# piyanon108/iGate4xSoftphoneDSP

Measured on AMD Instinct MI355X. Metric: Msamples/s G.711 decode+RMS, 65536ch@8kHz; %HBM roofline at 1/2/4/8 GPU, higher is better.
Workload: dtype u8

## Files before the change

### igate4xsoftphonedsp_amd/capi.py

```python
from __future__ import annotations

import ctypes as C
import os

import numpy as np

_PKG = os.path.dirname(os.path.abspath(__file__))
LIB_PATH = os.path.join(_PKG, "libigdsp.so")

ABI_VERSION = 3
PT_PCMU, PT_PCMA, PT_R2S = 0, 8, 123
SAMPLES_PER_FRAME = 160
MAX_PAYLOAD = 256
STAGE_DEPTH = 8
ENC_SUN16, ENC_G191 = 0, 1
FLAG_SILENT, FLAG_PROBE_D5, FLAG_CLIPPED, FLAG_EMPTY = 1, 2, 4, 8
FLAG_SATURATED = 0x10
BSS_VOTE_FRAMES = 10
PTT_RELEASE_FRAMES = 12
PTT_ON, PTT_PRESS, PTT_RELEASE, PTT_TAKEOVER = 1, 2, 4, 8
LINK_R2S_PERIOD_MS, LINK_MISS_TICKS = 200, 12
LINK_AUDIO_ON, LINK_AUDIO_OFF, LINK_MISSING, LINK_LATE, LINK_RECOVERED, LINK_CAME_UP = 1, 2, 4, 8, 0x10, 0x20
LINK_EVENT_DEFAULT = 0x37
LINK_UP, LINK_AUDIO, LINK_ALARMED = 1, 2, 4
# ... 72 lines not shown
RTP_V2, RTP_X, RTP_MARKER, RTP_ED137_OK, RTP_KEEPALIVE, RTP_METERED, RTP_RUNT, RTP_OVERSIZE = 1, 2, 4, 8, 16, 32, 64, 128
TX_CHAN = np.dtype(
    [("r2s_send_ms", "<u8"), ("ts", "<u4"), ("ssrc", "<u4"), ("keepalive_ms", "<i4"), ("packet_cnt", "<i4"), ("seq", "<u2"), ("pt", "u1"),
     ("first_r2s", "u1"), ("tx_slave", "u1"), ("rx_slave", "u1"), ("tx_slave_changed", "u1"), ("rx_slave_changed", "u1"),
     ("slave_count", "<i4"), ("ptt", "u1"), ("sql", "u1"), ("call_in", "u1"), ("call_recorder", "u1"), ("pttid", "u1"),
     ("pttpriority", "u1"), ("bssi", "u1"), ("calltype", "u1"), ("tx_run", "<i2"), ("level", "u1"), ("reserved0", "u1"),
     ("reserved", "<u4", (4,))],
    align=True,
)
TX_INFO = np.dtype([("ed137", "<u4"), ("size", "<u2"), ("flags", "u1"), ("level", "u1")], align=True)
TX_CT_IDLE, TX_CT_RX, TX_CT_TX = 1, 2, 4
TX_SENT, TX_KEEPALIVE_PT, TX_MARKER, TX_STALE_PAYLOAD, TX_LEVEL_VALID = 1, 2, 4, 8, 16
TX_CTL_PTT, TX_CTL_SQL, TX_CTL_MARK, TX_CTL_SET = 1, 2, 4, 0x80
TX_PACKET = np.dtype([("pkt", "<u8"), ("call_id", "<i4"), ("ed137", "<u4"), ("size", "<u2"), ("flags", "u1"), ("level", "u1")], align=True)
TX_MAX_N = 236
TX_SLOT = 256
AGGREGATE = np.dtype({
    "names": ["sumsq", "samples", "frames", "n_silent", "n_clipped", "byte_mean_sum", "peak_slot"],
    "formats": ["<u8", "<u8", "<u8", "<u8", "<u8", "<u8", ("<u8", (AGG_MAX_RANKS,))],
    "offsets": [128 * i for i in range(7)],
    "itemsize": 8 * AGG_WORDS,
})


class Level(C.Structure):
    _fields_ = [("byte_mean", C.c_uint8), ("flags", C.c_uint8), ("peak", C.c_uint16), ("rms", C.c_float),
                ("percent", C.c_int32), ("peak_hold", C.c_uint16), ("dropped", C.c_uint16), ("frames", C.c_uint32)]


class Window(C.Structure):
    _fields_ = [("gate_mode", C.c_uint32), ("probe_alarm", C.c_uint32), ("d_hold", C.c_void_p), ("d_gate", C.c_void_p),
                ("d_probe", C.c_void_p), ("d_work", C.c_void_p)]


class ChanProbe(C.Structure):
    _fields_ = [("run", C.c_uint32), ("alarms", C.c_uint32)]


IO_INPUT, IO_RECORD, IO_BULK = 0, 1, 2


class IoBuf(C.Structure):
    _fields_ = [("bytes", C.c_size_t), ("role", C.c_uint32), ("reserved", C.c_uint32), ("ptr", C.c_void_p)]


class IoReport(C.Structure):
    _fields_ = [("placed", C.c_uint32), ("bulk_spread", C.c_uint32), ("classes_found", C.c_uint32), ("chunks_explored", C.c_uint32),
                ("probes", C.c_uint32), ("reseeds", C.c_uint32), ("chunk_bytes", C.c_uint64), ("explored_bytes", C.c_uint64),
                ("probe_ms_same", C.c_float), ("probe_ms_other", C.c_float), ("setup_ms", C.c_float), ("settle_ms", C.c_float)]

    def as_dict(self):
        return {k: (round(getattr(self, k), 4) if isinstance(getattr(self, k), float) else getattr(self, k))
                for k, _ in self._fields_ if not k.startswith("reserved")}


class IgdspError(RuntimeError):
    def __init__(self, code: int, where: str, detail: str = ""):
        self.code = code
        super().__init__(f"{where} failed: {ERRORS.get(code, code)}" + (f" ({detail})" if detail else ""))


_vp, _u32, _u64, _i32, _int = C.c_void_p, C.c_uint32, C.c_uint64, C.c_int32, C.c_int
PROTOTYPES = [
    ("igdsp_abi_version", _int, []),
    ("igdsp_create", _int, [C.POINTER(_vp), _int, _u32]),
    ("igdsp_destroy", _int, [_vp]),
    ("igdsp_last_error", C.c_char_p, [_vp]),
    ("igdsp_device_info", _int, [_vp, C.POINTER(_int), C.POINTER(_int), C.c_char_p, C.c_size_t]),
    ("igdsp_map_call", _int, [_vp, _i32, _u32]),
    ("igdsp_unmap_call", _int, [_vp, _i32]),
    ("igdsp_on_rtp_frame", _int, [_vp, _i32, C.c_uint8, _vp, _u32]),
    ("igdsp_flush", _int, [_vp, C.POINTER(_u32)]),
    ("igdsp_flush_begin", _int, [_vp, C.POINTER(_u32)]),
    ("igdsp_flush_end", _int, [_vp, _int]),
    ("igdsp_set_ed137", _int, [_vp, _i32, _u32]),
    ("igdsp_set_gate_mode", _int, [_vp, _u32]),
    ("igdsp_get_probe", _int, [_vp, _u32, C.POINTER(ChanProbe)]),
    ("igdsp_poll", _int, [_vp, _u32, C.POINTER(Level)]),
    ("igdsp_poll_call", _int, [_vp, _i32, C.POINTER(Level)]),
    ("igdsp_reset_hold", _int, [_vp, _u32]),
    ("igdsp_get_hold", _int, [_vp, _u32, _vp]),
    ("igdsp_decode_meter", _int, [_vp, _vp, _vp, _vp, _u32, _u32, _u32, _vp, _vp, _vp, _u32, _vp]),
    ("igdsp_encode", _int, [_vp, _vp, _vp, _u32, _u32, _u32, _vp, _int, _vp]),
    ("igdsp_roundtrip_peakhold", _int, [_vp, _vp, _vp, _u32, _u32, _u32, _vp, _vp, _vp, _vp, _int, _vp]),
    ("igdsp_hold_update", _int, [_vp, _vp, _u32, _u32, _u32, _vp, _vp, _vp]),
    ("igdsp_hold_reset", _int, [_vp, _vp, _u32, _vp, _vp]),
    ("igdsp_agg_reset", _int, [_vp, _vp, _vp]),
    ("igdsp_depayload", _int, [_vp, _vp, _vp, _vp, _u32, _u32, _u32, _u32, _vp, _vp, _vp, _vp]),
    ("igdsp_decode_meter_rtp", _int, [_vp, _vp, _vp, _u32, _u32, _vp, _vp, _vp, _u32, _vp]),
    ("igdsp_decode_meter_packets", _int, [_vp, _vp, _vp, _vp, _u32, _u32, _u32, _u32, _vp, _vp, _vp, _u32, _vp]),
    ("igdsp_decode_meter_packets_mixed", _int, [_vp, _vp, _vp, _vp, _vp, _u32, _u32, _u32, _vp, _vp, _vp, _u32, _vp]),
    ("igdsp_window_work_bytes", C.c_size_t, [_u32]),
    ("igdsp_window_update", _int, [_vp, _vp, _vp, _vp, _u32, _u32, _u32, C.POINTER(Window), _vp]),
    ("igdsp_decode_meter_window", _int, [_vp, _u32, _vp, _vp, _vp, _vp, _u32, _u32, _u32, _u32, _vp, _vp, _vp, _u32, C.POINTER(Window), _vp]),
    ("igdsp_wav_expand", _int, [_vp, _vp, _u32, _u32, _u32, _u32, _vp, _u64, _vp]),
    ("igdsp_tx_chan_init", _int, [_vp, C.c_char_p, _int, C.c_uint8, _u32, C.c_uint16, _u32, _i32, _u64]),
    ("igdsp_tx_calltype_bits", _int, [C.c_char_p]),
    ("igdsp_tx_packetize", _int, [_vp, _vp, _vp, _vp, _u32, _u32, _u32, _u64, _u32, _vp, _vp, _vp, _u32, _vp, _vp, _int, _vp]),
    ("igdsp_tx_open", _int, [_vp, _i32, C.c_char_p, _int, _i32, _u64]),
    ("igdsp_tx_close", _int, [_vp, _i32]),
    ("igdsp_tx_set_ptt", _int, [_vp, _i32, _int, _int, _int]),
    ("igdsp_tx_set_sql", _int, [_vp, _i32, _int, _int, _i32]),
    ("igdsp_tx_set_ptt_id", _int, [_vp, _i32, _int]),
    ("igdsp_tx_set_slave", _int, [_vp, _i32, _int, _int]),
    ("igdsp_tx_set_recorder", _int, [_vp, _i32, _int]),
    ("igdsp_tx_set_calltype", _int, [_vp, _i32, C.c_char_p]),
# ... 448 lines not shown
        self._ck(self.L.igdsp_tx_results(self.h, C.byref(p), C.byref(n)), "igdsp_tx_results")
        if n.value == 0:
            return np.zeros(0, TX_PACKET), np.zeros((0, TX_SLOT), np.uint8)
        ent = np.frombuffer((C.c_uint8 * (n.value * TX_PACKET.itemsize)).from_address(p.value), TX_PACKET).copy()
        pk = np.frombuffer((C.c_uint8 * (n.value * TX_SLOT)).from_address(int(ent["pkt"][0])), np.uint8).reshape(n.value, TX_SLOT).copy()
        return ent, pk

    def tx_get_chan(self, call_id: int) -> np.ndarray:
        out = np.zeros((), TX_CHAN)
        self._ck(self.L.igdsp_tx_get_chan(self.h, call_id, out.ctypes.data_as(_vp)), "igdsp_tx_get_chan")
        return out

    def tx_counts(self, call_id: int):
        r, d = _u32(), _u32()
        self._ck(self.L.igdsp_tx_counts(self.h, call_id, C.byref(r), C.byref(d)), "igdsp_tx_counts")
        return r.value, d.value

    @staticmethod
    def window(hold, gate_mode=GATE_ALWAYS, gate=None, probe=None, work=None, probe_alarm=0) -> Window:
        w = Window(gate_mode, probe_alarm, _ptr(hold), _ptr(gate), _ptr(probe), _ptr(work))
        w._keep = (hold, gate, probe, work)
        return w

    def window_work_bytes(self, C_: int) -> int:
        return int(self.L.igdsp_window_work_bytes(C_))

    def window_update(self, stats, C_, F_, n, win: Window, info=None, length=None, stream=None):
        self._ck(self.L.igdsp_window_update(self.h, _ptr(stats), _ptr(info), _ptr(length), C_, F_, n, C.byref(win), stream), "igdsp_window_update")

    def decode_meter_window(self, layout, packets, sizes, codec, radio, C_, F_, stride, hdr, stats, win: Window, info=None, agg=None, rank=0, stream=None):
        self._ck(self.L.igdsp_decode_meter_window(self.h, layout, _ptr(packets), _ptr(sizes), _ptr(codec), _ptr(radio), C_, F_, stride, hdr,
                                                  _ptr(stats), _ptr(info), _ptr(agg), rank, C.byref(win), stream), "igdsp_decode_meter_window")

    def wav_expand(self, payload, C_, F_, n, files, file_stride, rate=8000, stream=None):
        self._ck(self.L.igdsp_wav_expand(self.h, _ptr(payload), C_, F_, n, rate, _ptr(files), file_stride, stream), "igdsp_wav_expand")

    def g726_reorder(self, d_in, d_out, n_bytes, mode, stream=None):
        self._ck(self.L.igdsp_g726_reorder(self.h, _ptr(d_in), _ptr(d_out), n_bytes, mode, stream), "igdsp_g726_reorder")

    def gen_uniform(self, out, n_bytes, seed=0x20241218, first_byte=0, stream=None):
        self._ck(self.L.igdsp_gen_uniform(self.h, _ptr(out), n_bytes, seed, first_byte, stream), "igdsp_gen_uniform")

    def stream_read(self, src, n_bytes, sink, stream=None):
        self._ck(self.L.igdsp_stream_read(self.h, _ptr(src), n_bytes, _ptr(sink), stream), "igdsp_stream_read")

    def dev_alloc(self, nbytes: int) -> int:
        p = _vp()
        self._ck(self.L.igdsp_dev_alloc(self.h, C.byref(p), nbytes), "igdsp_dev_alloc")
        return p.value

    def dev_free(self, ptr: int):
        self._ck(self.L.igdsp_dev_free(self.h, ptr), "igdsp_dev_free")

    def dev_memset(self, ptr, value: int, nbytes: int):
        self._ck(self.L.igdsp_dev_memset(self.h, _ptr(ptr), value, nbytes), "igdsp_dev_memset")

    def io_alloc(self, bufs, explore_limit_bytes: int = 0):
        arr = (IoBuf * len(bufs))()
        for a, (nb, role) in zip(arr, bufs):
            a.bytes, a.role = int(nb), int(role)
        st, rep = _vp(), IoReport()
        self._ck(self.L.igdsp_io_alloc(self.h, arr, len(bufs), explore_limit_bytes, C.byref(st), C.byref(rep)), "igdsp_io_alloc")
        return IoSet(self, st), [a.ptr for a in arr], rep.as_dict()

    def sync(self, stream=None):
        self._ck(self.L.igdsp_sync(self.h, stream), "igdsp_sync")

    def probe_placement(self, buf, n_bytes, out=None, reps=10, stream=None) -> float:
        ms = C.c_float(0)
        self._ck(self.L.igdsp_probe_placement(self.h, _ptr(buf), n_bytes, _ptr(out), reps, C.byref(ms), stream), "igdsp_probe_placement")
        return float(ms.value)

    def timer(self):
        return Timer(self)


class IoSet:

    def __init__(self, ctx: Context, handle):
        self.ctx, self.h = ctx, handle

    def close(self):
        if self.h and self.ctx.h:
            self.ctx.L.igdsp_io_free(self.ctx.h, self.h)
        self.h = None


class DevView:

    def __init__(self, ptr: int, nbytes: int):
        self.__cuda_array_interface__ = {"shape": (int(nbytes),), "typestr": "|u1", "data": (int(ptr), False), "version": 3, "strides": None}


def as_tensor(ptr: int, nbytes: int, dtype=None, shape=None):
    import torch

    t = torch.as_tensor(DevView(ptr, nbytes), device="cuda")
    if dtype is not None:
        t = t.view(dtype)
    return t.view(shape) if shape is not None else t


class Timer:
    def __init__(self, ctx: Context):
        self.ctx = ctx
        self.t = _vp()
# ... 18 lines not shown
```

### igate4xsoftphonedsp_amd/csrc/igdsp_capi_ctx.hip

```cpp
#include "igdsp_ctx.h"

#include <algorithm>
#include <atomic>
#include <cmath>
#include <cstdlib>
#include <cstring>
#include <mutex>
#include <new>
#include <vector>

using namespace igdsp;
using igdsp_rx::kSlot;
using igdsp_rx::kStageDepth;

extern "C" {

int igdsp_abi_version(void) { return IGDSP_ABI_VERSION; }

int igdsp_create(igdsp_ctx **out, int device, uint32_t max_channels)
{
    if (!out || max_channels == 0 || max_channels > (1u << 24)) return IGDSP_EINVAL;
    *out = nullptr;
    int count = 0;
    if (hipGetDeviceCount(&count) != hipSuccess || count <= 0 || device < 0 || device >= count) return IGDSP_ENODEV;
    hipDeviceProp_t prop;
    if (hipGetDeviceProperties(&prop, device) != hipSuccess) return IGDSP_ENODEV;
    if (std::strncmp(prop.gcnArchName, "gfx950", 6) != 0) return IGDSP_ENODEV;
    if (hipSetDevice(device) != hipSuccess) return IGDSP_ENODEV;

    igdsp_ctx *ctx = new (std::nothrow) igdsp_ctx();
    if (!ctx) return IGDSP_ENOMEM;
    ctx->device = device;
    ctx->cus = prop.multiProcessorCount;
    ctx->name = prop.name;
    ctx->max_channels = max_channels;
    ctx->direct = std::vector<std::atomic<uint32_t>>(kDirectCalls);
    for (auto &d : ctx->direct) d.store(kNoChan, std::memory_order_relaxed);
    const size_t max_frames = (size_t)max_channels * kStageDepth;
    ctx->up_bytes = igdsp_rx::upload_layout(max_frames, max_channels).total;
    bool ok = hipStreamCreateWithFlags(&ctx->stream, hipStreamNonBlocking) == hipSuccess;
    ok = ok && hipEventCreateWithFlags(&ctx->flush_done, hipEventDisableTiming) == hipSuccess;
    for (int i = 0; i < igdsp_rx::RingMem::kArrays; ++i)
        ok = ok && hipHostMalloc(ctx->ring.array(i), igdsp_rx::RingMem::bytes(max_channels, i), hipHostMallocDefault) == hipSuccess;
    if (ok) ctx->rx.init(max_channels, ctx->ring);
    ok = ok && hipHostMalloc((void **)&ctx->h_up, ctx->up_bytes, hipHostMallocDefault) == hipSuccess;
    for (uint32_t i = 0; i < 2; ++i) {
        igdsp_rx::Published &pb = ctx->pub.set(i);
        ok = ok && hipHostMalloc((void **)&pb.last, max_channels * sizeof(igdsp_frame_stats), hipHostMallocDefault) == hipSuccess;
        ok = ok && hipHostMalloc((void **)&pb.hold, max_channels * sizeof(igdsp_chan_hold), hipHostMallocDefault) == hipSuccess;
        ok = ok && hipHostMalloc((void **)&pb.probe, max_channels * sizeof(igdsp_chan_probe), hipHostMallocDefault) == hipSuccess;
    }
    ok = ok && hipMalloc((void **)&ctx->d_up, ctx->up_bytes) == hipSuccess;
    ok = ok && hipMalloc((void **)&ctx->d_stats, 2 * max_frames * sizeof(igdsp_frame_stats)) == hipSuccess;
    ok = ok && hipMalloc((void **)&ctx->d_last, max_channels * sizeof(igdsp_frame_stats)) == hipSuccess;
    ok = ok && hipMalloc((void **)&ctx->d_hold, max_channels * sizeof(igdsp_chan_hold)) == hipSuccess;
    ok = ok && hipMalloc((void **)&ctx->d_probe, max_channels * sizeof(igdsp_chan_probe)) == hipSuccess;
    ok = ok && hipMalloc((void **)&ctx->d_queues, kQueueRing * 32u * sizeof(uint32_t)) == hipSuccess;
    ok = ok && hipMemset(ctx->d_queues, 0, kQueueRing * 32u * sizeof(uint32_t)) == hipSuccess;
    ok = ok && hipMemset(ctx->d_last, 0, max_channels * sizeof(igdsp_frame_stats)) == hipSuccess;
    ok = ok && hipMemset(ctx->d_probe, 0, max_channels * sizeof(igdsp_chan_probe)) == hipSuccess;
    if (const char *e = std::getenv("IGDSP_GLOBAL_QUEUE")) ctx->global_queue = std::atoi(e) != 0;
    if (const char *e = std::getenv("IGDSP_IO_SPARE_CHUNKS")) ctx->io_spare_cap = (size_t)std::max(0, std::atoi(e));
    if (!ok) {
        igdsp_destroy(ctx);
        return IGDSP_ENOMEM;
    }
    if (init_device_attributes() != hipSuccess) {
        igdsp_destroy(ctx);
        return IGDSP_EDEVICE;
    }
    bool up = launch_hold_reset(ctx->d_hold, max_channels, nullptr, ctx->stream) == hipSuccess;
    for (uint32_t i = 0; i < 2; ++i) {
        igdsp_rx::Published &pb = ctx->pub.set(i);
        std::memset(pb.last, 0, max_channels * sizeof(igdsp_frame_stats));
        std::memset(pb.probe, 0, max_channels * sizeof(igdsp_chan_probe));
        up = up && hipMemcpyAsync(pb.hold, ctx->d_hold, max_channels * sizeof(igdsp_chan_hold), hipMemcpyDeviceToHost, ctx->stream) == hipSuccess;
    }
    if (!up || hipStreamSynchronize(ctx->stream) != hipSuccess) {
        igdsp_destroy(ctx);
        return IGDSP_EDEVICE;
    }
    ctx->pool = make_pool(max_channels);
    *out = ctx;
    return IGDSP_OK;
}

int igdsp_destroy(igdsp_ctx *ctx)
{
    if (!ctx) return IGDSP_OK;
    ctx->pool.reset();
    if (ctx->device >= 0) (void)hipSetDevice(ctx->device);
    igdsp_tx_drop(ctx);
    igdsp_io_drop_spares(ctx);
    if (ctx->stream) { (void)hipStreamSynchronize(ctx->stream); (void)hipStreamDestroy(ctx->stream); }
    if (ctx->flush_done) (void)hipEventDestroy(ctx->flush_done);
    for (int i = 0; i < igdsp_rx::RingMem::kArrays; ++i) if (*ctx->ring.array(i)) (void)hipHostFree(*ctx->ring.array(i));
    const igdsp_rx::Published &p0 = ctx->pub.set(0), &p1 = ctx->pub.set(1);
    void *hosts[] = {ctx->h_up, p0.last, p0.hold, p0.probe, p1.last, p1.hold, p1.probe};
    for (void *p : hosts) if (p) (void)hipHostFree(p);
    void *devs[] = {ctx->d_up, ctx->d_stats, ctx->d_last, ctx->d_hold, ctx->d_probe, ctx->d_queues, ctx->d_enc_tab[0], ctx->d_enc_tab[1]};
    for (void *p : devs) if (p) (void)hipFree(p);
    delete ctx;
    return IGDSP_OK;
}

const char *igdsp_last_error(const igdsp_ctx *ctx) { return ctx ? ctx->err.c_str() : ""; }

int igdsp_device_info(const igdsp_ctx *ctx, int *device, int *compute_units, char *name, size_t name_len)
{
    if (!ctx) return IGDSP_EINVAL;
    if (device) *device = ctx->device;
    if (compute_units) *compute_units = ctx->cus;
    if (name && name_len) { std::strncpy(name, ctx->name.c_str(), name_len - 1); name[name_len - 1] = 0; }
    return IGDSP_OK;
}
// ... 153 lines not shown
    igdsp_frame_stats s;
    uint16_t peak_hold = 0;
    ctx->pub.read([&](const igdsp_rx::Published &p) { s = p.last[channel]; peak_hold = p.hold[channel].peak_hold; });
    out->byte_mean = s.byte_mean;
    out->flags = s.flags;
    out->peak = s.peak;
    out->rms = s.rms;
    out->percent = (int32_t)(float)(((double)s.rms * 100.0) / (double)IGDSP_METER_FULL_SCALE);
    out->peak_hold = peak_hold;
    out->dropped = (uint16_t)std::min<uint32_t>(ctx->rx.frames_dropped(channel), 65535u);
    out->frames = ctx->rx.frames_seen(channel);
    return IGDSP_OK;
}

int igdsp_poll_call(igdsp_ctx *ctx, int32_t call_id, igdsp_level *out)
{
    if (!ctx || !out) return IGDSP_EINVAL;
    const uint32_t ch = lookup(ctx, call_id);
    if (ch == kNoChan) return IGDSP_ENOENT;
    return igdsp_poll(ctx, ch, out);
}

int igdsp_reset_hold(igdsp_ctx *ctx, uint32_t channel)
{
    if (!ctx) return IGDSP_EINVAL;
    if (channel != 0xFFFFFFFFu && channel >= ctx->max_channels) return IGDSP_ERANGE;
    std::lock_guard<std::mutex> g(ctx->flush_mu);
    if (int rc = flush_end_locked(ctx, 1)) return rc;
    HIP_TRY(ctx, hipSetDevice(ctx->device));
    const uint32_t c0 = (channel == 0xFFFFFFFFu) ? 0 : channel;
    const uint32_t cn = (channel == 0xFFFFFFFFu) ? ctx->max_channels : 1;
    HIP_TRY(ctx, launch_hold_reset(ctx->d_hold + c0, cn, nullptr, ctx->stream));
    HIP_TRY(ctx, hipMemcpyAsync(ctx->pub.back().hold + c0, ctx->d_hold + c0, cn * sizeof(igdsp_chan_hold), hipMemcpyDeviceToHost, ctx->stream));
    HIP_TRY(ctx, hipStreamSynchronize(ctx->stream));
    ctx->pub.rewrite_front([&](igdsp_rx::Published &front, const igdsp_rx::Published &back) {
        std::memcpy(front.hold + c0, back.hold + c0, cn * sizeof(igdsp_chan_hold));
    });
    return IGDSP_OK;
}

int igdsp_get_hold(igdsp_ctx *ctx, uint32_t channel, igdsp_chan_hold *out)
{
    if (!ctx || !out) return IGDSP_EINVAL;
    if (channel >= ctx->max_channels) return IGDSP_ERANGE;
    ctx->pub.read([&](const igdsp_rx::Published &p) { *out = p.hold[channel]; });
    return IGDSP_OK;
}

int igdsp_get_probe(igdsp_ctx *ctx, uint32_t channel, igdsp_chan_probe *out)
{
    if (!ctx || !out) return IGDSP_EINVAL;
    if (channel >= ctx->max_channels) return IGDSP_ERANGE;
    ctx->pub.read([&](const igdsp_rx::Published &p) { *out = p.probe[channel]; });
    return IGDSP_OK;
}

int igdsp_dev_alloc(igdsp_ctx *ctx, void **d_ptr, size_t bytes)
{
    if (!ctx || !d_ptr) return IGDSP_EINVAL;
    *d_ptr = nullptr;
    if (bytes == 0) return IGDSP_OK;
    if (hipSetDevice(ctx->device) != hipSuccess) return IGDSP_ENODEV;
    hipError_t e = hipMalloc(d_ptr, bytes);
    return e == hipSuccess ? IGDSP_OK : fail(ctx, IGDSP_ENOMEM, "hipMalloc", e);
}

int igdsp_dev_free(igdsp_ctx *ctx, void *d_ptr)
{
    if (!ctx) return IGDSP_EINVAL;
    if (!d_ptr) return IGDSP_OK;
    HIP_TRY(ctx, hipSetDevice(ctx->device));
    HIP_TRY(ctx, hipFree(d_ptr));
    return IGDSP_OK;
}

int igdsp_dev_alloc_far(igdsp_ctx *ctx, void **d_ptr, size_t bytes, const void *d_in, size_t in_bytes, uint32_t max_tries,
                        size_t spacer_bytes, float *ms_first, float *ms_kept)
{
    if (!ctx || !d_ptr || !d_in || bytes == 0 || in_bytes < 10240u || max_tries == 0) return IGDSP_EINVAL;
    *d_ptr = nullptr;
    if (hipSetDevice(ctx->device) != hipSuccess) return IGDSP_ENODEV;
    if (spacer_bytes == 0) spacer_bytes = (size_t)12 << 30;
    const size_t cand_bytes = std::max(bytes, in_bytes / 10u + 4096u);
    std::vector<void *> spacers;
    void *best = nullptr;
    float t_best = 0.f, t_first = 0.f;
    int rc = IGDSP_OK;
    for (uint32_t k = 0; k < max_tries; ++k) {
        if (k > 0) {
            void *sp = nullptr;
            if (hipMalloc(&sp, spacer_bytes) != hipSuccess) { (void)hipGetLastError(); break; }
            spacers.push_back(sp);
        }
        void *cand = nullptr;
        if (hipMalloc(&cand, cand_bytes) != hipSuccess) { (void)hipGetLastError(); break; }
        float ms = 0.f;
        rc = igdsp_probe_placement(ctx, d_in, in_bytes, cand, 6, &ms, nullptr);
        if (rc != IGDSP_OK) { (void)hipFree(cand); break; }
        if (k == 0) t_first = ms;
        if (best == nullptr || ms < t_best) {
            if (best) (void)hipFree(best);
            best = cand; t_best = ms;
        } else {
            (void)hipFree(cand);
        }
        if (t_best < 0.92f * t_first) break;
    }
    for (void *sp : spacers) (void)hipFree(sp);
    if (rc != IGDSP_OK) { if (best) (void)hipFree(best); return rc; }
    if (!best) return fail(ctx, IGDSP_ENOMEM, "igdsp_dev_alloc_far");
    *d_ptr = best;
    if (ms_first) *ms_first = t_first;
    if (ms_kept) *ms_kept = t_best;
    return IGDSP_OK;
}

int igdsp_copy_h2d(igdsp_ctx *ctx, void *d_dst, const void *h_src, size_t bytes)
{
    if (!ctx || (bytes && (!d_dst || !h_src))) return IGDSP_EINVAL;
    HIP_TRY(ctx, hipSetDevice(ctx->device));
    HIP_TRY(ctx, hipMemcpy(d_dst, h_src, bytes, hipMemcpyHostToDevice));
    return IGDSP_OK;
}

int igdsp_copy_d2h(igdsp_ctx *ctx, void *h_dst, const void *d_src, size_t bytes)
// ... 73 lines not shown
```

### igate4xsoftphonedsp_amd/csrc/igdsp_ctx.h

```cpp
#pragma once
#include "igdsp_args.h"
#include "igdsp_internal.h"
#include "igdsp_rxstage.h"
#include "igdsp_snappool.h"

#include <atomic>
#include <cstdio>
#include <mutex>
#include <string>
#include <unordered_map>
#include <vector>

namespace {
constexpr uint32_t kNoChan = 0xFFFFFFFFu;
constexpr int32_t kDirectCalls = 1 << 16;
}

struct igdsp_ctx {
    int device = -1;
    int cus = 0;
    std::string name;
    uint32_t max_channels = 0;
    hipStream_t stream = nullptr;
    int variant = 0;
    std::string err;

    struct IoRange { const char *base; size_t bytes; };
    std::vector<IoRange> spread_ranges;
    std::vector<hipMemGenericAllocationHandle_t> io_spare[4];
    size_t io_spare_chunk = 0;
    size_t io_spare_cap = 16;
    uint32_t io_epoch = 0;
    std::mutex io_mu;
    bool is_spread(const void *p)
    {
        std::lock_guard<std::mutex> g(io_mu);
        for (const auto &r : spread_ranges) if ((const char *)p >= r.base && (const char *)p < r.base + r.bytes) return true;
        return false;
    }

    std::vector<std::atomic<uint32_t>> direct;
    std::unordered_map<int32_t, uint32_t> far;
    std::mutex far_mu;

    igdsp_rx::RingMem ring;
    igdsp_rx::Stager rx;
    std::atomic<uint32_t> gate_mode{IGDSP_GATE_ALWAYS};

    uint8_t *h_up = nullptr, *d_up = nullptr;
    size_t up_bytes = 0;
    igdsp_frame_stats *d_stats = nullptr;
    igdsp_frame_stats *d_last = nullptr;
    igdsp_chan_hold *d_hold = nullptr;
    igdsp_chan_probe *d_probe = nullptr;
    igdsp_rx::PublishedSet pub;
    hipEvent_t flush_done = nullptr;
    bool flush_open = false;
    uint32_t flush_nch = 0;
    std::mutex flush_mu;

    std::unique_ptr<igdsp::SnapshotPool> pool;

    struct TxSide;
    std::atomic<TxSide *> tx{nullptr};
    std::mutex tx_init_mu;

    uint32_t *d_queues = nullptr;
    uint8_t *d_enc_tab[2] = {nullptr, nullptr};
    std::once_flag enc_once[2];
    hipStream_t queue_owner[64];
    uint32_t queue_launches[64];
    uint32_t queue_used = 0;
    uint32_t queue_hint = 0;
    std::atomic_flag queue_lk = ATOMIC_FLAG_INIT;
    bool global_queue = true;
};
namespace {
constexpr uint32_t kQueueRing = 64;
const hipStream_t kFreeQueue = reinterpret_cast<hipStream_t>(~(uintptr_t)0);
}

void igdsp_io_drop_spares(igdsp_ctx *ctx);
void igdsp_tx_drop(igdsp_ctx *ctx);

static inline uint32_t lookup(igdsp_ctx *ctx, int32_t call_id)
{
// ... 82 lines not shown
```

### igate4xsoftphonedsp_amd/csrc/igdsp_io.hip

```cpp
#include "igdsp_ctx.h"

#include <algorithm>
#include <chrono>
#include <thread>
#include <cmath>
#include <cstdlib>
#include <cstring>
#include <new>

using namespace igdsp;

struct igdsp_io_set {
    struct Map { void *va = nullptr; size_t bytes = 0; std::vector<hipMemGenericAllocationHandle_t> handles; std::vector<uint8_t> cls; };
    uint32_t epoch = 0;
    std::vector<Map> maps;
    std::vector<void *> plain;
    size_t chunk = 0;
    int device = 0;
};

namespace {

constexpr size_t kSrcChunks = 10;

struct Chunk {
    hipMemGenericAllocationHandle_t h{};
    float tA = -1.f;
    float tB = -1.f;
    bool used = false;
    bool mapped = false;
    bool in_src = false;
    int cls = -1;
};

struct Source { void *va = nullptr; size_t n = 0; std::vector<size_t> idx; };

struct Explorer {
    igdsp_ctx *ctx = nullptr;
    hipStream_t s = nullptr;
    size_t chunk = 0;
    size_t va_align = 0;
    hipMemAllocationProp prop{};
    hipMemAccessDesc acc{};
    void *cand_va = nullptr;
    bool debug = false;
    hipEvent_t ea = nullptr, eb = nullptr;
    std::vector<Chunk> chunks;
    std::vector<Source> sources;
    size_t limit_chunks = 0;
    size_t probe_n = 0;
    uint32_t probes = 0;

    bool open(igdsp_ctx *c, size_t n) { ctx = c; s = c->stream; probe_n = n; return hipEventCreate(&ea) == hipSuccess && hipEventCreate(&eb) == hipSuccess; }
    bool ensure(size_t idx)
    {
        while (chunks.size() <= idx) {
            if (chunks.size() >= limit_chunks) return false;
            Chunk c;
            if (hipMemCreate(&c.h, chunk, &prop, 0) != hipSuccess) { (void)hipGetLastError(); return false; }
            chunks.push_back(c);
        }
        return true;
    }
    void unmap_scratch(size_t idx)
    {
        if (chunks[idx].mapped) { (void)hipMemUnmap((char *)cand_va + idx * chunk, chunk); chunks[idx].mapped = false; }
    }
    bool time_pair(const void *rd, void *dst, float *ms)
    {
        hipError_t e = hipSuccess;
        for (int i = 0; i < 2 && e == hipSuccess; ++i) e = launch_stream_rw(cfg_of(ctx, s), rd, probe_n, dst, s);
        if (e == hipSuccess) e = hipEventRecord(ea, s);
        for (int i = 0; i < 4 && e == hipSuccess; ++i) e = launch_stream_rw(cfg_of(ctx, s), rd, probe_n, dst, s);
        if (e == hipSuccess) e = hipEventRecord(eb, s);
        if (e == hipSuccess) e = hipEventSynchronize(eb);
// ... 271 lines not shown
            P.b = cb; P.c = cc; P.split = true; P.thrB = thrB; P.thrC = thrC;
        }
        X.drop_source(srcB);
    }
    bool run(igdsp_ctx *ctx, igdsp_io_set *set, const IoKnobs &kn, size_t limit)
    {
        igdsp_io_drop_spares(ctx);
        { std::lock_guard<std::mutex> g(ctx->io_mu); set->epoch = ++ctx->io_epoch; ctx->io_spare_chunk = X.chunk; }
        X.limit_chunks = limit / X.chunk; X.debug = kn.debug;
        ok = hipMemAddressReserve(&X.cand_va, X.limit_chunks * X.chunk, X.va_align, nullptr, 0) == hipSuccess && X.open(ctx, probe_bytes(X.chunk));
        classify(L.bulk_chunks >= 4 && !kn.no_spread, ctx->io_spare_cap);
        R.chunks_explored = (uint32_t)X.chunks.size(); R.explored_bytes = (uint64_t)X.chunks.size() * X.chunk; R.probes = X.probes;
        (void)hipGetLastError();
        return ok;
    }
    void classify(bool want_spread, size_t spare_cap)
    {
        std::vector<size_t> first;
        for (size_t k = 0; k < kSrcChunks && ok; ++k) { ok = X.ensure(k); first.push_back(k); }
        ok = ok && X.make_source(first, &srcA);
        {
            float t = 0.f;
            if (ok && X.ensure(kSrcChunks)) { for (int k = 0; k < 28 && ok; ++k) ok = X.probe(kSrcChunks, X.sources[srcA], &t, "warm"); }
        }
        if (ok) survey(false);
        for (int attempt = 0; attempt < 2 && ok && tmax > 1.02f * tmin && tmax < kPure * tmin; ++attempt)
            if (!reseed_A()) break;
        R.probe_ms_same = tmax; R.probe_ms_other = tmin;
        if (!ok || !(tmax > kBimodal * tmin)) return;
        R.classes_found = 2;
        P.fast = kNear * tmin; P.slow = tmax / kNear;
        if (L.in_chunks > kSrcChunks) walk(0, L.in_chunks - kSrcChunks, [this](size_t i) { return !X.chunks[i].in_src && timeA(i) && X.chunks[i].tA > P.slow; }, P.a);
        const size_t outs = L.rec_chunks + L.bulk_chunks;
        walk(0, want_spread ? std::max<size_t>(outs + kSrcChunks, 4 * kSrcChunks) : outs, [this](size_t i) { return fast_A(i); }, P.b);
        if (ok && want_spread && P.b.size() >= kSrcChunks + outs - L.bulk_chunks / 2) split_BC();
        if (ok && !want_spread && spare_cap > 0) {
            const size_t need0 = (L.in_chunks > kSrcChunks ? L.in_chunks - kSrcChunks : 0) + spare_cap, need1 = L.rec_chunks + L.bulk_chunks + spare_cap;
            size_t cnt0 = 0, cnt1 = 0;
            for (const auto &c : X.chunks) if (!c.in_src && c.tA >= 0.f) { if (c.tA > P.slow) ++cnt0; else if (c.tA < P.fast) ++cnt1; }
            size_t budget = 4 * spare_cap;
            for (size_t k = 0; k < X.chunks.size() && ok && budget > 0 && (cnt0 < need0 || cnt1 < need1); ++k) {
                Chunk &c = X.chunks[k];
                if (c.in_src || c.tA >= 0.f) continue;
                if (!timeA(k)) break;
                --budget;
                if (c.tA > P.slow) ++cnt0; else if (c.tA < P.fast) ++cnt1;
            }
        }
        if (!ok) return;
        P.a.insert(P.a.begin(), X.sources[srcA].idx.begin(), X.sources[srcA].idx.end());
        X.drop_source(srcA);
    }
};
int plain_path(igdsp_ctx *ctx, igdsp_io_buf *bufs, uint32_t n_bufs, igdsp_io_set *set)
{
    for (uint32_t i = 0; i < n_bufs; ++i) {
        if (hipMalloc(&bufs[i].ptr, bufs[i].bytes) != hipSuccess) { (void)hipGetLastError(); bufs[i].ptr = nullptr; return fail(ctx, IGDSP_ENOMEM, "igdsp_io_alloc: hipMalloc"); }
        set->plain.push_back(bufs[i].ptr);
    }
    return IGDSP_OK;
}
int reserve_ranges(igdsp_ctx *ctx, const igdsp_io_buf *bufs, uint32_t n_bufs, size_t va_align, igdsp_io_set *set, Layout &L)
{
    const size_t chunk = set->chunk;
    set->maps.resize(n_bufs); L.nch.resize(n_bufs);
    for (uint32_t role = 0; role < 3; ++role)
        for (uint32_t i = 0; i < n_bufs; ++i) if (bufs[i].role == role) L.order.push_back(i);
    for (uint32_t i = 0; i < n_bufs; ++i) {
        L.nch[i] = (bufs[i].bytes + chunk - 1) / chunk;
        auto &m = set->maps[i];
        m.bytes = L.nch[i] * chunk;
        if (hipMemAddressReserve(&m.va, m.bytes, va_align, nullptr, 0) != hipSuccess) { (void)hipGetLastError(); m.va = nullptr; return fail(ctx, IGDSP_ENOMEM, "igdsp_io_alloc: hipMemAddressReserve"); }
        if (bufs[i].role == IGDSP_IO_INPUT) { L.in_chunks += L.nch[i]; L.in_bytes += bufs[i].bytes; if (L.in0 < 0 || L.nch[i] > L.nch[L.in0]) L.in0 = (int)i; continue; }
        if (L.out0 < 0) L.out0 = (int)i;
        if (bufs[i].role == IGDSP_IO_RECORD) L.rec_chunks += L.nch[i]; else L.bulk_chunks += L.nch[i];
    }
    return IGDSP_OK;
}
int publish(igdsp_ctx *ctx, igdsp_io_buf *bufs, uint32_t n_bufs, const igdsp_io_set *set, bool spread)
{
    for (uint32_t i = 0; i < n_bufs; ++i) bufs[i].ptr = set->maps[i].va;
    if (!spread) return IGDSP_OK;
    std::lock_guard<std::mutex> g(ctx->io_mu);
    for (uint32_t i = 0; i < n_bufs; ++i)
        if (bufs[i].role == IGDSP_IO_BULK) ctx->spread_ranges.push_back({(const char *)set->maps[i].va, set->maps[i].bytes});
    return IGDSP_OK;
}
constexpr int kNotServed = 1;
int from_spares(igdsp_ctx *ctx, igdsp_io_buf *bufs, uint32_t n_bufs, const Layout &L, igdsp_io_set *set, const hipMemAccessDesc &acc, igdsp_io_report &R)
{
    const bool want_spread = L.bulk_chunks >= 4;
    const size_t second = want_spread ? L.bulk_chunks / 2 : 0, first = L.rec_chunks + L.bulk_chunks - second;
    std::unique_lock<std::mutex> g(ctx->io_mu);
    auto &S = ctx->io_spare;
    if (ctx->io_spare_chunk != set->chunk || S[0].size() < L.in_chunks || S[1].size() + S[2].size() < first || S[3].size() < second) return kNotServed;
    const uint32_t epoch = ctx->io_epoch;
    const int pref = want_spread ? 2 : 1;
    for (uint32_t i : L.order) {
        auto &m = set->maps[i];
        const size_t h2 = (bufs[i].role == IGDSP_IO_BULK && want_spread) ? L.nch[i] / 2 : 0;
        for (size_t k = 0; k < L.nch[i]; ++k) {
            const int from = bufs[i].role == IGDSP_IO_INPUT ? 0 : (k >= L.nch[i] - h2 && !S[3].empty()) ? 3
                           : !S[pref].empty() ? pref : !S[3 - pref].empty() ? 3 - pref : 3;
            m.handles.push_back(S[from].back()); m.cls.push_back((uint8_t)from); S[from].pop_back();
        }
    }
// ... 70 lines not shown
        if (c.tA > P.slow) c.cls = 0;
        else if (c.tA < P.fast) c.cls = !P.split ? 1 : (c.tB > P.thrB ? 2 : ((c.tB >= 0.f && c.tB < P.thrC) ? 3 : -1));
    }
    std::lock_guard<std::mutex> g(ctx->io_mu);
    for (auto &c : X.chunks)
        if (!c.used && !c.in_src && c.cls >= 0 && ctx->io_spare[c.cls].size() < ctx->io_spare_cap) { ctx->io_spare[c.cls].push_back(c.h); c.used = true; }
}
bool map_fresh(igdsp_io_set::Map &m, size_t nch, size_t chunk, const hipMemAllocationProp &prop, const hipMemAccessDesc &acc)
{
    const size_t have = m.handles.size();
    std::vector<hipMemGenericAllocationHandle_t> hs;
    bool ok = true;
    hipMemGenericAllocationHandle_t h;
    for (size_t k = have; k < nch && ok; ++k) if ((ok = hipMemCreate(&h, chunk, &prop, 0) == hipSuccess)) hs.push_back(h);
    ok = ok && map_chunks(m, chunk, hs, have, acc);
    m.handles.insert(m.handles.end(), hs.begin(), hs.end());
    m.cls.resize(m.handles.size(), 255);
    return ok;
}
float settle_ref(Explorer &X, const Layout &L, const igdsp_io_set *set, size_t *n)
{
    if (L.in0 < 0 || L.out0 < 0) return 0.f;
    *n = std::min(X.probe_n, std::min(L.nch[L.in0] * set->chunk, 10 * (L.nch[L.out0] * set->chunk - 4096)) / 10240 * 10240);
    const size_t keep = X.probe_n; X.probe_n = *n;
    float t = 0.f, t_ref = 0.f;
    const void *rd = set->maps[L.in0].va; void *wr = set->maps[L.out0].va;
    if (*n >= ((size_t)256 << 20) && X.time_pair(rd, wr, &t) && X.time_pair(rd, wr, &t)) t_ref = t;
    X.probe_n = keep;
    return t_ref;
}
float settle(igdsp_ctx *ctx, const Layout &L, const igdsp_io_set *set, size_t n, float t_ref, size_t released_chunks, bool debug)
{
    Explorer Y;
    const auto w0 = std::chrono::steady_clock::now();
    if (Y.open(ctx, n)) {
        const float min_wait = std::min(6000.f, (float)((double)released_chunks * (double)set->chunk / 25e9 * 1e3));
        int quiet = 0;
        for (;;) {
            float t = 0.f; if (!Y.time_pair(set->maps[L.in0].va, set->maps[L.out0].va, &t)) break;
            quiet = t <= 1.012f * t_ref ? quiet + 1 : 0;
            const float waited = std::chrono::duration<float, std::milli>(std::chrono::steady_clock::now() - w0).count();
            if (debug) std::fprintf(stderr, "[igdsp_io] settle: %.4f ms against %.4f before the release (%.0f of >= %.0f ms)\n", t, t_ref, waited, min_wait);
            if ((quiet >= 2 && waited >= min_wait) || waited > 8000.f) break;
            std::this_thread::sleep_for(std::chrono::milliseconds(50));
        }
    }
    const float ms = std::chrono::duration<float, std::milli>(std::chrono::steady_clock::now() - w0).count();
    Y.cleanup();
    return ms;
}
int place(igdsp_ctx *ctx, igdsp_io_buf *bufs, uint32_t n_bufs, size_t explore_limit_bytes, const IoKnobs &kn, igdsp_io_set *set,
          Explorer &X, igdsp_io_report &R)
{
    int vmm = 0;
    if (hipDeviceGetAttribute(&vmm, hipDeviceAttributeVirtualMemoryManagementSupported, ctx->device) != hipSuccess) { (void)hipGetLastError(); vmm = 0; }
    if (!vmm || kn.plain) return plain_path(ctx, bufs, n_bufs, set);
    X.prop.type = hipMemAllocationTypePinned; X.prop.location.type = hipMemLocationTypeDevice; X.prop.location.id = ctx->device;
    X.acc.location = X.prop.location; X.acc.flags = hipMemAccessFlagsProtReadWrite;
    size_t gran = 0;
    if (hipMemGetAllocationGranularity(&gran, &X.prop, hipMemAllocationGranularityRecommended) != hipSuccess || gran == 0) { (void)hipGetLastError(); return plain_path(ctx, bufs, n_bufs, set); }
    const size_t chunk = (((size_t)128 << 20) + gran - 1) / gran * gran;
    X.chunk = set->chunk = R.chunk_bytes = chunk;
    X.va_align = kn.align_mib >= 0 ? (size_t)kn.align_mib << 20 : chunk;
    Layout L;
    if (const int rc = reserve_ranges(ctx, bufs, n_bufs, X.va_align, set, L)) return rc;
    size_t free_b = 0, total_b = 0; (void)hipMemGetInfo(&free_b, &total_b);
    const double frac = kn.frac_set ? kn.limit_frac : (L.bulk_chunks >= 4 ? 0.85 : 0.5);
    const size_t limit = std::min(explore_limit_bytes ? explore_limit_bytes : (size_t)(frac * (double)free_b), (size_t)(0.9 * (double)free_b));
    const bool want_place = L.in_bytes >= ((size_t)512 << 20) && ((L.rec_chunks + L.bulk_chunks) > 0 || L.in_chunks > kSrcChunks) && limit / chunk >= 4 * kSrcChunks;
    const int spared = want_place ? from_spares(ctx, bufs, n_bufs, L, set, X.acc, R) : kNotServed;
    if (spared != kNotServed) return spared;
    Search S{X, L, kn.stride, R};
    bool ok = !want_place || S.run(ctx, set, kn, limit);
    if (ok && (!S.P.b.empty() || (L.rec_chunks + L.bulk_chunks == 0 && !S.P.a.empty()))) ok = hand_out(X, S.P, bufs, n_bufs, L, set, R);
    size_t settle_n = 0;
    const float t_ref = R.placed ? settle_ref(X, L, set, &settle_n) : 0.f;
    if (R.placed) keep_spares(ctx, X, S.P);
    const size_t released_chunks = (size_t)std::count_if(X.chunks.begin(), X.chunks.end(), [](const Chunk &c) { return !c.used; });
    X.cleanup();
    for (uint32_t i : L.order)
        if (ok && set->maps[i].handles.size() < L.nch[i]) ok = map_fresh(set->maps[i], L.nch[i], chunk, X.prop, X.acc);
    if (!ok) { (void)hipGetLastError(); return fail(ctx, IGDSP_ENOMEM, "igdsp_io_alloc: mapping chunks"); }
    publish(ctx, bufs, n_bufs, set, R.bulk_spread);
    if (kn.settle && t_ref > 0.f) R.settle_ms = settle(ctx, L, set, settle_n, t_ref, released_chunks, kn.debug);
    if (kn.debug && R.placed) { Explorer Y; if (Y.open(ctx, probe_bytes(chunk))) debug_check(Y, bufs, n_bufs, L, set, true); Y.cleanup(); }
    return IGDSP_OK;
}

}

void igdsp_io_drop_spares(igdsp_ctx *ctx)
{
    std::vector<hipMemGenericAllocationHandle_t> gone;
    std::unique_lock<std::mutex> g(ctx->io_mu);
    for (auto &v : ctx->io_spare) { gone.insert(gone.end(), v.begin(), v.end()); v.clear(); }
    g.unlock();
    for (auto h : gone) (void)hipMemRelease(h);
    (void)hipGetLastError();
}

extern "C" {

int igdsp_io_free(igdsp_ctx *ctx, igdsp_io_set *set)
{
    if (!ctx) return IGDSP_EINVAL;
    if (!set) return IGDSP_OK;
    (void)hipSetDevice(set->device);
    (void)hipDeviceSynchronize();
    {
        std::lock_guard<std::mutex> g(ctx->io_mu);
        for (auto &m : set->maps)
            for (size_t k = 0; k < ctx->spread_ranges.size();)
                if (ctx->spread_ranges[k].base == (const char *)m.va) ctx->spread_ranges.erase(ctx->spread_ranges.begin() + (long)k); else ++k;
    }
    for (auto &m : set->maps) {
        if (!m.va) continue;
        for (size_t i = 0; i < m.handles.size(); ++i) (void)hipMemUnmap((char *)m.va + i * set->chunk, set->chunk);
        std::vector<hipMemGenericAllocationHandle_t> gone;
        std::unique_lock<std::mutex> g(ctx->io_mu);
        for (size_t i = 0; i < m.handles.size(); ++i) {
            const uint8_t c = i < m.cls.size() ? m.cls[i] : 255;
            if (c < 4 && set->epoch == ctx->io_epoch && set->chunk == ctx->io_spare_chunk && ctx->io_spare[c].size() < ctx->io_spare_cap) ctx->io_spare[c].push_back(m.handles[i]);
            else gone.push_back(m.handles[i]);
        }
        g.unlock();
        for (auto h : gone) (void)hipMemRelease(h);
    }
    for (void *p : set->plain) if (p) (void)hipFree(p);
    (void)hipGetLastError();
    delete set;
    return IGDSP_OK;
}

int igdsp_internal_vmm_remap_check(igdsp_ctx *ctx, int mode, int *bytes)
{
    if (!ctx || !bytes) return IGDSP_EINVAL;
    HIP_TRY(ctx, hipSetDevice(ctx->device));
    hipMemAllocationProp prop{};
    prop.type = hipMemAllocationTypePinned;
    prop.location.type = hipMemLocationTypeDevice;
    prop.location.id = ctx->device;
    hipMemAccessDesc acc{};
    acc.location = prop.location;
    acc.flags = hipMemAccessFlagsProtReadWrite;
    size_t gran = 0;
    HIP_TRY(ctx, hipMemGetAllocationGranularity(&gran, &prop, hipMemAllocationGranularityRecommended));
    const size_t sz = std::max<size_t>(gran, (size_t)64 << 20);
    hipMemGenericAllocationHandle_t X, Y;
    void *v = nullptr, *wx = nullptr, *wy = nullptr;
    HIP_TRY(ctx, hipMemCreate(&X, sz, &prop, 0));
    HIP_TRY(ctx, hipMemCreate(&Y, sz, &prop, 0));
    HIP_TRY(ctx, hipMemAddressReserve(&v, sz, 0, nullptr, 0));
    HIP_TRY(ctx, hipMemAddressReserve(&wx, sz, 0, nullptr, 0));
    HIP_TRY(ctx, hipMemAddressReserve(&wy, sz, 0, nullptr, 0));
// ... 59 lines not shown
```

Before: 5.993 million.

## Route large dev_alloc buffers through VMM chunk placement search

Large allocations made with igdsp_dev_alloc (at least one 128 MiB chunk) now go through the same VMM physical-chunk placement machinery used by io_alloc. Chunks come from the spare pool by class, or from a fresh probe search, and are mapped into a contiguous VA range; freeing returns the handles to the spare pool. The aim is to place bulk buffers in physical memory classes with better HBM bandwidth, rather than wherever hipMalloc puts them. The cost is setup time for probing and settling, added complexity, and a fallback to hipMalloc when placement fails.

```diff
diff --git a/igate4xsoftphonedsp_amd/capi.py b/igate4xsoftphonedsp_amd/capi.py
--- a/igate4xsoftphonedsp_amd/capi.py
+++ b/igate4xsoftphonedsp_amd/capi.py
@@ -148,6 +148,14 @@
     def as_dict(self):
         return {k: (round(getattr(self, k), 4) if isinstance(getattr(self, k), float) else getattr(self, k))
                 for k, _ in self._fields_ if not k.startswith("reserved")}
+
+
+class DevAllocInfo(C.Structure):
+    _fields_ = [("placed", C.c_uint32), ("reason", C.c_uint32), ("cls", C.c_uint32), ("epoch", C.c_uint32), ("chunks", C.c_uint32),
+                ("from_spares", C.c_uint32), ("probes", C.c_uint32), ("classes_found", C.c_uint32), ("chunk_bytes", C.c_uint64),
+                ("explored_bytes", C.c_uint64), ("setup_ms", C.c_float), ("settle_ms", C.c_float)]
+    REASONS = ("placed", "small", "off", "no_vmm", "no_class", "vmm_failed")
+    as_dict = IoReport.as_dict
 
 
 class IgdspError(RuntimeError):
@@ -702,6 +710,13 @@
     def dev_free(self, ptr: int):
         self._ck(self.L.igdsp_dev_free(self.h, ptr), "igdsp_dev_free")
 
+    def dev_alloc_info(self, ptr: int) -> dict:
+        fn = self.L.igdsp_internal_dev_alloc_info
+        fn.restype, fn.argtypes = _int, [_vp, _vp, C.POINTER(DevAllocInfo)]
+        info = DevAllocInfo()
+        self._ck(fn(self.h, ptr, C.byref(info)), "igdsp_internal_dev_alloc_info")
+        return dict(info.as_dict(), reason=DevAllocInfo.REASONS[info.reason])
+
     def dev_memset(self, ptr, value: int, nbytes: int):
         self._ck(self.L.igdsp_dev_memset(self.h, _ptr(ptr), value, nbytes), "igdsp_dev_memset")
 
diff --git a/igate4xsoftphonedsp_amd/csrc/igdsp_capi_ctx.hip b/igate4xsoftphonedsp_amd/csrc/igdsp_capi_ctx.hip
--- a/igate4xsoftphonedsp_amd/csrc/igdsp_capi_ctx.hip
+++ b/igate4xsoftphonedsp_amd/csrc/igdsp_capi_ctx.hip
@@ -61,6 +61,7 @@
     ok = ok && hipMemset(ctx->d_probe, 0, max_channels * sizeof(igdsp_chan_probe)) == hipSuccess;
     if (const char *e = std::getenv("IGDSP_GLOBAL_QUEUE")) ctx->global_queue = std::atoi(e) != 0;
     if (const char *e = std::getenv("IGDSP_IO_SPARE_CHUNKS")) ctx->io_spare_cap = (size_t)std::max(0, std::atoi(e));
+    if (const char *e = std::getenv("IGDSP_DEV_ALLOC_PLACE")) ctx->dev_place = std::atoi(e) != 0;
     if (!ok) {
         igdsp_destroy(ctx);
         return IGDSP_ENOMEM;
@@ -320,25 +321,6 @@
     if (!ctx || !out) return IGDSP_EINVAL;
     if (channel >= ctx->max_channels) return IGDSP_ERANGE;
     ctx->pub.read([&](const igdsp_rx::Published &p) { *out = p.probe[channel]; });
-    return IGDSP_OK;
-}
-
-int igdsp_dev_alloc(igdsp_ctx *ctx, void **d_ptr, size_t bytes)
-{
-    if (!ctx || !d_ptr) return IGDSP_EINVAL;
-    *d_ptr = nullptr;
-    if (bytes == 0) return IGDSP_OK;
-    if (hipSetDevice(ctx->device) != hipSuccess) return IGDSP_ENODEV;
-    hipError_t e = hipMalloc(d_ptr, bytes);
-    return e == hipSuccess ? IGDSP_OK : fail(ctx, IGDSP_ENOMEM, "hipMalloc", e);
-}
-
-int igdsp_dev_free(igdsp_ctx *ctx, void *d_ptr)
-{
-    if (!ctx) return IGDSP_EINVAL;
-    if (!d_ptr) return IGDSP_OK;
-    HIP_TRY(ctx, hipSetDevice(ctx->device));
-    HIP_TRY(ctx, hipFree(d_ptr));
     return IGDSP_OK;
 }
 
diff --git a/igate4xsoftphonedsp_amd/csrc/igdsp_ctx.h b/igate4xsoftphonedsp_amd/csrc/igdsp_ctx.h
--- a/igate4xsoftphonedsp_amd/csrc/igdsp_ctx.h
+++ b/igate4xsoftphonedsp_amd/csrc/igdsp_ctx.h
@@ -16,6 +16,28 @@
 constexpr int32_t kDirectCalls = 1 << 16;
 }
 
+#define IGDSP_DEV_PLACED        0u
+#define IGDSP_DEV_SMALL         1u
+#define IGDSP_DEV_OFF           2u
+#define IGDSP_DEV_NO_VMM        3u
+#define IGDSP_DEV_NO_CLASS      4u
+#define IGDSP_DEV_VMM_FAILED    5u
+struct igdsp_dev_alloc_info {
+    uint32_t placed;
+    uint32_t reason;
+    uint32_t cls;
+    uint32_t epoch;
+    uint32_t chunks;
+    uint32_t from_spares;
+    uint32_t probes;
+    uint32_t classes_found;
+    uint64_t chunk_bytes;
+    uint64_t explored_bytes;
+    float setup_ms;
+    float settle_ms;
+};
+extern "C" int igdsp_internal_dev_alloc_info(igdsp_ctx *ctx, const void *d_ptr, igdsp_dev_alloc_info *out);
+
 struct igdsp_ctx {
     int device = -1;
     int cus = 0;
@@ -32,6 +54,16 @@
     size_t io_spare_cap = 16;
     uint32_t io_epoch = 0;
     std::mutex io_mu;
+    struct DevAlloc {
+        size_t chunk = 0;
+        std::vector<hipMemGenericAllocationHandle_t> handles;
+        uint32_t epoch = 0;
+        igdsp_dev_alloc_info info{};
+    };
+    std::unordered_map<const void *, DevAlloc> dev_allocs;
+    bool dev_place = true;
+    int dev_last_cls = -1;
+    uint32_t dev_last_epoch = 0;
     bool is_spread(const void *p)
     {
         std::lock_guard<std::mutex> g(io_mu);
diff --git a/igate4xsoftphonedsp_amd/csrc/igdsp_io.hip b/igate4xsoftphonedsp_amd/csrc/igdsp_io.hip
--- a/igate4xsoftphonedsp_amd/csrc/igdsp_io.hip
+++ b/igate4xsoftphonedsp_amd/csrc/igdsp_io.hip
@@ -21,6 +21,8 @@
 
 namespace {
 
+constexpr size_t kChunkBytes = (size_t)128 << 20;
+constexpr size_t kDevPlaceMinBytes = kChunkBytes;
 constexpr size_t kSrcChunks = 10;
 
 struct Chunk {
@@ -398,6 +400,19 @@
         X.drop_source(srcA);
     }
 };
+bool open_vmm(igdsp_ctx *ctx, const IoKnobs &kn, Explorer &X)
+{
+    int vmm = 0;
+    if (hipDeviceGetAttribute(&vmm, hipDeviceAttributeVirtualMemoryManagementSupported, ctx->device) != hipSuccess) { (void)hipGetLastError(); vmm = 0; }
+    if (!vmm) return false;
+    X.prop.type = hipMemAllocationTypePinned; X.prop.location.type = hipMemLocationTypeDevice; X.prop.location.id = ctx->device;
+    X.acc.location = X.prop.location; X.acc.flags = hipMemAccessFlagsProtReadWrite;
+    size_t gran = 0;
+    if (hipMemGetAllocationGranularity(&gran, &X.prop, hipMemAllocationGranularityRecommended) != hipSuccess || gran == 0) { (void)hipGetLastError(); return false; }
+    X.chunk = (kChunkBytes + gran - 1) / gran * gran;
+    X.va_align = kn.align_mib >= 0 ? (size_t)kn.align_mib << 20 : X.chunk;
+    return true;
+}
 int plain_path(igdsp_ctx *ctx, igdsp_io_buf *bufs, uint32_t n_bufs, igdsp_io_set *set)
 {
     for (uint32_t i = 0; i < n_bufs; ++i) {
@@ -574,16 +589,8 @@
 int place(igdsp_ctx *ctx, igdsp_io_buf *bufs, uint32_t n_bufs, size_t explore_limit_bytes, const IoKnobs &kn, igdsp_io_set *set,
           Explorer &X, igdsp_io_report &R)
 {
-    int vmm = 0;
-    if (hipDeviceGetAttribute(&vmm, hipDeviceAttributeVirtualMemoryManagementSupported, ctx->device) != hipSuccess) { (void)hipGetLastError(); vmm = 0; }
-    if (!vmm || kn.plain) return plain_path(ctx, bufs, n_bufs, set);
-    X.prop.type = hipMemAllocationTypePinned; X.prop.location.type = hipMemLocationTypeDevice; X.prop.location.id = ctx->device;
-    X.acc.location = X.prop.location; X.acc.flags = hipMemAccessFlagsProtReadWrite;
-    size_t gran = 0;
-    if (hipMemGetAllocationGranularity(&gran, &X.prop, hipMemAllocationGranularityRecommended) != hipSuccess || gran == 0) { (void)hipGetLastError(); return plain_path(ctx, bufs, n_bufs, set); }
-    const size_t chunk = (((size_t)128 << 20) + gran - 1) / gran * gran;
-    X.chunk = set->chunk = R.chunk_bytes = chunk;
-    X.va_align = kn.align_mib >= 0 ? (size_t)kn.align_mib << 20 : chunk;
+    if (kn.plain || !open_vmm(ctx, kn, X)) return plain_path(ctx, bufs, n_bufs, set);
+    const size_t chunk = set->chunk = R.chunk_bytes = X.chunk;
     Layout L;
     if (const int rc = reserve_ranges(ctx, bufs, n_bufs, X.va_align, set, L)) return rc;
     size_t free_b = 0, total_b = 0; (void)hipMemGetInfo(&free_b, &total_b);
@@ -609,6 +616,130 @@
     return IGDSP_OK;
 }
 
+constexpr int8_t kDevNext[5][4] = {{0, 2, 1, 3}, {2, 1, 3, -1}, {0, -1, -1, -1}, {3, 0, -1, -1}, {0, 2, -1, -1}};
+
+void dev_unmap(void *va, size_t n, size_t chunk)
+{
+    for (size_t k = 0; k < n; ++k) (void)hipMemUnmap((char *)va + k * chunk, chunk);
+    (void)hipGetLastError();
+}
+void dev_give_back(igdsp_ctx *ctx, const igdsp_ctx::DevAlloc &d)
+{
+    std::vector<hipMemGenericAllocationHandle_t> gone;
+    {
+        std::lock_guard<std::mutex> g(ctx->io_mu);
+        const uint32_t c = d.info.cls;
+        for (auto h : d.handles) {
+            if (c < 4 && d.epoch == ctx->io_epoch && d.chunk == ctx->io_spare_chunk && ctx->io_spare[c].size() < ctx->io_spare_cap) ctx->io_spare[c].push_back(h);
+            else gone.push_back(h);
+        }
+    }
+    for (auto h : gone) (void)hipMemRelease(h);
+    (void)hipGetLastError();
+}
+int dev_from_spares(igdsp_ctx *ctx, Explorer &X, size_t n, void **va, igdsp_ctx::DevAlloc &d)
+{
+    {
+        std::lock_guard<std::mutex> g(ctx->io_mu);
+        if (ctx->io_spare_chunk != X.chunk) return kNotServed;
+        const int last = ctx->dev_last_epoch == ctx->io_epoch ? ctx->dev_last_cls : -1;
+        int cls = -1;
+        for (int8_t c : kDevNext[last + 1]) if (c >= 0 && cls < 0 && ctx->io_spare[c].size() >= n) cls = c;
+        if (cls < 0) return kNotServed;
+        auto &S = ctx->io_spare[cls];
+        d.handles.assign(S.end() - (long)n, S.end());
+        S.resize(S.size() - n);
+        d.epoch = ctx->io_epoch; d.info.cls = (uint32_t)cls;
+        ctx->dev_last_cls = cls; ctx->dev_last_epoch = d.epoch;
+    }
+    igdsp_io_set::Map m;
+    bool ok = hipMemAddressReserve(&m.va, n * X.chunk, X.va_align, nullptr, 0) == hipSuccess;
+    if (!ok) m.va = nullptr;
+    ok = ok && map_chunks(m, X.chunk, d.handles, 0, X.acc);
+    if (ok) { *va = m.va; d.info.from_spares = 1; return IGDSP_OK; }
+    (void)hipGetLastError();
+    if (m.va) dev_unmap(m.va, n, X.chunk);
+    dev_give_back(ctx, d);
+    d.handles.clear();
+    d.info.reason = IGDSP_DEV_VMM_FAILED;
+    return IGDSP_ENOMEM;
+}
+int dev_search(igdsp_ctx *ctx, const IoKnobs &kn, Explorer &X, size_t n, void **va, igdsp_ctx::DevAlloc &d)
+{
+    igdsp_dev_alloc_info &I = d.info;
+    Layout L;
+    L.in_chunks = n;
+    L.bulk_chunks = 2 * std::max<size_t>(2, std::min(std::max<size_t>(n, 4), ctx->io_spare_cap));
+    size_t free_b = 0, total_b = 0; (void)hipMemGetInfo(&free_b, &total_b);
+    const size_t limit = (size_t)(std::min(kn.frac_set ? kn.limit_frac : 0.5, 0.9) * (double)free_b);
+    I.reason = IGDSP_DEV_NO_CLASS;
+    if (limit / X.chunk < 4 * kSrcChunks) return kNotServed;
+    igdsp_io_set label; label.chunk = X.chunk;
+    igdsp_io_report R = {};
+    Search S{X, L, kn.stride, R};
+    const bool ok = S.run(ctx, &label, kn, limit);
+    I.probes = R.probes; I.explored_bytes = R.explored_bytes; I.classes_found = R.classes_found;
+    if (!ok) { I.reason = IGDSP_DEV_VMM_FAILED; return kNotServed; }
+    if (R.classes_found < 2 || S.P.a.size() < n) return kNotServed;
+    for (size_t i = 0; i < X.chunks.size(); ++i) X.unmap_scratch(i);
+    for (size_t k = 0; k < n; ++k) d.handles.push_back(X.chunks[S.P.a[k]].h);
+    igdsp_io_set::Map m;
+    bool mapped = hipMemAddressReserve(&m.va, n * X.chunk, X.va_align, nullptr, 0) == hipSuccess;
+    if (!mapped) m.va = nullptr;
+    mapped = mapped && map_chunks(m, X.chunk, d.handles, 0, X.acc);
+    if (!mapped) {
+        (void)hipGetLastError();
+        if (m.va) dev_unmap(m.va, n, X.chunk);
+        d.handles.clear();
+        I.reason = IGDSP_DEV_VMM_FAILED;
+        return kNotServed;
+    }
+    for (size_t k = 0; k < n; ++k) X.chunks[S.P.a[k]].used = true;
+    d.epoch = label.epoch; I.cls = 0;
+    Layout SL; SL.nch = {n, n}; SL.in0 = 0; SL.out0 = 1;
+    igdsp_io_set sset; sset.chunk = X.chunk; sset.maps.resize(2); sset.maps[0].va = sset.maps[1].va = m.va;
+    size_t settle_n = 0;
+    const float t_ref = kn.settle ? settle_ref(X, SL, &sset, &settle_n) : 0.f;
+    keep_spares(ctx, X, S.P);
+    const size_t released = (size_t)std::count_if(X.chunks.begin(), X.chunks.end(), [](const Chunk &c) { return !c.used; });
+    X.cleanup();
+    if (kn.settle && released > 0) {
+        if (t_ref > 0.f) I.settle_ms = settle(ctx, SL, &sset, settle_n, t_ref, released, kn.debug);
+        else {
+            I.settle_ms = std::min(6000.f, (float)((double)released * (double)X.chunk / 25e9 * 1e3));
+            std::this_thread::sleep_for(std::chrono::microseconds((long)(I.settle_ms * 1e3f)));
+        }
+    }
+    {
+        std::lock_guard<std::mutex> g(ctx->io_mu);
+        if (ctx->io_epoch == d.epoch) { ctx->dev_last_cls = 0; ctx->dev_last_epoch = d.epoch; }
+    }
+    *va = m.va;
+    return IGDSP_OK;
+}
+void dev_place(igdsp_ctx *ctx, size_t bytes, void **va, igdsp_ctx::DevAlloc &d)
+{
+    igdsp_dev_alloc_info &I = d.info;
+    I.cls = 255;
+    I.reason = IGDSP_DEV_OFF;
+    if (!ctx->dev_place || ctx->io_spare_cap == 0) return;
+    const auto t_start = std::chrono::steady_clock::now();
+    const IoKnobs kn;
+    Explorer X; X.ctx = ctx; X.s = ctx->stream;
+    I.reason = IGDSP_DEV_NO_VMM;
+    if (open_vmm(ctx, kn, X)) {
+        const size_t n = (bytes + X.chunk - 1) / X.chunk;
+        d.chunk = I.chunk_bytes = X.chunk;
+        int rc = dev_from_spares(ctx, X, n, va, d);
+        if (rc == kNotServed) rc = dev_search(ctx, kn, X, n, va, d);
+        if (rc == IGDSP_OK) { I.placed = 1; I.reason = IGDSP_DEV_PLACED; I.chunks = (uint32_t)n; I.epoch = d.epoch; }
+        else { *va = nullptr; I.cls = 255; }
+    }
+    X.cleanup();
+    I.setup_ms = std::chrono::duration<float, std::milli>(std::chrono::steady_clock::now() - t_start).count();
+    if (kn.debug) std::fprintf(stderr, "[igdsp_io] dev_alloc %zu bytes: placed %u reason %u class %u spares %u probes %u setup %.1f ms\n", bytes, I.placed, I.reason, I.cls, I.from_spares, I.probes, I.setup_ms);
+}
+
 }
 
 void igdsp_io_drop_spares(igdsp_ctx *ctx)
@@ -622,6 +753,52 @@
 }
 
 extern "C" {
+
+int igdsp_dev_alloc(igdsp_ctx *ctx, void **d_ptr, size_t bytes)
+{
+    if (!ctx || !d_ptr) return IGDSP_EINVAL;
+    *d_ptr = nullptr;
+    if (bytes == 0) return IGDSP_OK;
+    if (hipSetDevice(ctx->device) != hipSuccess) return IGDSP_ENODEV;
+    const bool large = bytes >= kDevPlaceMinBytes;
+    igdsp_ctx::DevAlloc d;
+    if (large) dev_place(ctx, bytes, d_ptr, d);
+    if (!*d_ptr) {
+        const hipError_t e = hipMalloc(d_ptr, bytes);
+        if (e != hipSuccess) { *d_ptr = nullptr; return fail(ctx, IGDSP_ENOMEM, "hipMalloc", e); }
+    }
+    if (large) { std::lock_guard<std::mutex> g(ctx->io_mu); ctx->dev_allocs[*d_ptr] = std::move(d); }
+    return IGDSP_OK;
+}
+
+int igdsp_dev_free(igdsp_ctx *ctx, void *d_ptr)
+{
+    if (!ctx) return IGDSP_EINVAL;
+    if (!d_ptr) return IGDSP_OK;
+    HIP_TRY(ctx, hipSetDevice(ctx->device));
+    igdsp_ctx::DevAlloc d;
+    {
+        std::lock_guard<std::mutex> g(ctx->io_mu);
+        auto it = ctx->dev_allocs.find(d_ptr);
+        if (it != ctx->dev_allocs.end()) { d = std::move(it->second); ctx->dev_allocs.erase(it); }
+    }
+    if (d.handles.empty()) { HIP_TRY(ctx, hipFree(d_ptr)); return IGDSP_OK; }
+    (void)hipDeviceSynchronize();
+    dev_unmap(d_ptr, d.handles.size(), d.chunk);
+    dev_give_back(ctx, d);
+    return IGDSP_OK;
+}
+
+int igdsp_internal_dev_alloc_info(igdsp_ctx *ctx, const void *d_ptr, igdsp_dev_alloc_info *out)
+{
+    if (!ctx || !out) return IGDSP_EINVAL;
+    *out = igdsp_dev_alloc_info{};
+    out->reason = IGDSP_DEV_SMALL; out->cls = 255;
+    std::lock_guard<std::mutex> g(ctx->io_mu);
+    auto it = ctx->dev_allocs.find(d_ptr);
+    if (it != ctx->dev_allocs.end()) *out = it->second.info;
+    return IGDSP_OK;
+}
 
 int igdsp_io_free(igdsp_ctx *ctx, igdsp_io_set *set)
 {
```

After: 5.974 million, median of 2. No clear change (-0.3%).
